# nadeemlab/DeepLIIF

Measured on AMD Instinct MI355X. Metric: 512x512 tiles/s train-step (5G+5D), higher is better.
Workload: dtype bf16; 1 GPU; DeepLIIF train step, 5x Resnet-9block G + 5x NLayerD(n=4), GAN+SmoothL1+Adam (BASELINE configs[2] per GPU); tile=512x512x3, batch_per_gpu=8, global_batch=8, norm=instance, precision_policy=bf16, parallelism=dp1, rccl_ranks=1, backend=nccl, streams=3

## Files before the change

deepliif_amd/csrc/conv_gemm.hip:

```cpp
#include "common.h"
#include <stdlib.h>

#include "conv_args.h"

bool w4_eligible(const ConvArgs &a);
int launch_conv_w4(const ConvArgs &a0, hipStream_t stream);
bool w4x3_eligible(const ConvArgs &a);
int launch_conv_w4x3(const ConvArgs &a0, hipStream_t stream);
bool s2f_eligible(const ConvArgs &a);
int s2f_stats_chunks(const ConvArgs &a);
int launch_conv_s2f(const ConvArgs &a0, hipStream_t stream);
bool d1g_eligible(const ConvArgs &a);
int launch_conv_d1g(const ConvArgs &a0, hipStream_t stream);
bool d1_eligible(const ConvArgs &a);
int launch_conv_d1(const ConvArgs &a0, hipStream_t stream);
bool dot_fwd_eligible(const ConvArgs &a);
bool dot_dgrad_eligible(const ConvArgs &a);
int launch_conv_dot(const ConvArgs &a, bool fwd, hipStream_t stream);
bool s2u_eligible(const ConvArgs &a);
int s2u_stats_chunks(const ConvArgs &a);
int launch_conv_s2u(const ConvArgs &a0, hipStream_t stream);
bool s2d_eligible(const ConvArgs &a);
int s2d_stats_chunks(const ConvArgs &a);
int launch_conv_s2d(const ConvArgs &a0, hipStream_t stream);
// ... 527 lines not shown
                    red[(wm * 2 + 0) * BN + c] = st1[i][r];
                    red[(wm * 2 + 1) * BN + c] = st2[i][r];
                }
        }
        __syncthreads();
        const int m0 = tm * BM;
        const int n = m0 / HWq;
        const int chunk = ((m0 - n * HWq) / BM) * a.n_phase + phase;
        for (int c = tid; c < BN; c += NW * 64) {
            const int co = tn * BN + c;
            if (co < a.Co) {
                float s1 = 0.f, s2 = 0.f;
#pragma unroll
                for (int w = 0; w < WM; ++w) { s1 += red[(w * 2 + 0) * BN + c]; s2 += red[(w * 2 + 1) * BN + c]; }
                float *o = a.stats_part + ((size_t)(n * a.stats_nchunks + chunk) * 2) * a.Co + co;
                o[0] = s1;
                o[a.Co] = s2;
            }
        }
    }
}


template <int BM, int BN, int BK, int WM, int WN, bool UTAP, bool STAG = false, int ABL = 0>
__global__ void __launch_bounds__(WM * WN * 64) conv_gemm_glds_kernel(const ConvArgs a) {
    constexpr int NW = WM * WN;
    constexpr int CPR = BK / 8;
    constexpr int RPI = 64 / CPR;
    constexpr int X_INS = (BM + NW * RPI - 1) / (NW * RPI);
    constexpr int W_INS = (BN + NW * RPI - 1) / (NW * RPI);
    constexpr int PM = BM / WM, PN = BN / WN, FM = PM / 16, FN = PN / 16;
    constexpr int XT = BM * BK, WT = BN * BK, BUF = XT + WT;
    static_assert(NW == 4 || NW == 8, "4 or 8 waves");

    extern __shared__ __attribute__((aligned(16))) char smem_raw[];
    bf16_t *smem = reinterpret_cast<bf16_t *>(smem_raw);
    int16_t *tap_lds = reinterpret_cast<int16_t *>(smem + 2 * BUF);
    int *tapd_lds = reinterpret_cast<int *>(tap_lds + DL_MAX_TAPS);

    const int tid = threadIdx.x;
    const int lane = tid & 63, wave = __builtin_amdgcn_readfirstlane(tid >> 6);
    const int wm = wave % WM, wn = wave / WM;

    const int bid = xcd_remap(blockIdx.x, gridDim.x);
    const int tn = bid % a.tiles_n, tm = bid / a.tiles_n;
    const int phase = blockIdx.y / a.splitk, ks = blockIdx.y % a.splitk;
    const int tap0 = a.phase_tap_begin[phase];
    const int ntaps = a.phase_tap_begin[phase + 1] - tap0;
    const int kbase = a.phase_kbase[phase];
    const int nk_total = (ntaps * a.Ci + 63) / 64 * 64 / BK;
    const int nk_per = (nk_total + a.splitk - 1) / a.splitk;
    const int kt_begin = ks * nk_per;
    const int kt_end = min(nk_total, kt_begin + nk_per);

    if (tid < DL_MAX_TAPS) {
        const int16_t tp = a.taps[tid];
        tap_lds[tid] = tp;
        tapd_lds[tid] = ((int)(int8_t)(tp & 0xff) * a.Wi + (int)(int8_t)((tp >> 8) & 0xff)) * a.in_pstride;
    }

// ... 18 lines not shown
        x_wi0[i] = wq * a.in_step;
        x_chunk[i] = swz_chunk<CPR>(row, lcp);
        x_ptr[i] = in + ((size_t)(n * a.Hi + x_hi0[i]) * a.Wi + x_wi0[i]) * (size_t)a.in_pstride + x_chunk[i] * 8;
        unsigned long long mk = 0;
        if (UTAP && x_ok[i]) {
            for (int t = 0; t < ntaps; ++t) {
                const int16_t tp = a.taps[tap0 + t];
                const int hi = x_hi0[i] + (int)(int8_t)(tp & 0xff), wi = x_wi0[i] + (int)(int8_t)((tp >> 8) & 0xff);
                if (a.pad_mode == DL_PAD_REFLECT || (((unsigned)hi < (unsigned)a.Hi) && ((unsigned)wi < (unsigned)a.Wi))) mk |= 1ull << t;
            }
        }
        x_mask[i] = mk;
    }
    const bf16_t *w_ptr[W_INS];
#pragma unroll
    for (int i = 0; i < W_INS; ++i) {
        const int row = (wave * W_INS + i) * RPI + lrow;
        const int c = swz_chunk<CPR>(row, lcp);
        w_ptr[i] = a.w_hi + (size_t)(tn * BN + (row < BN ? row : 0)) * a.w_kstride + kbase + c * 8;
    }

    int is_tl = 0, is_ch = 0;
    int tapd_next = 0;
    auto issue_tile = [&](int kt, int buf) {
        bf16_t *base = smem + buf * BUF;
        size_t wk;
        if constexpr (UTAP) {
            const int tl = is_tl;
            const ptrdiff_t delta = (ptrdiff_t)tapd_next + is_ch;
            wk = (size_t)tl * a.Ci + is_ch;
            if (a.k_order) { if (++is_tl == ntaps) { is_tl = 0; is_ch += BK; } }
            else { is_ch += BK; if (is_ch == a.Ci) { is_ch = 0; ++is_tl; } }
            tapd_next = tapd_lds[tap0 + min(is_tl, ntaps - 1)];
#pragma unroll
            for (int i = 0; i < X_INS; ++i) {
                const int row0 = (wave * X_INS + i) * RPI;
                if (row0 < BM) {
                    const bool ok = (x_mask[i] >> tl) & 1ull;
                    const bf16_t *src = ok ? x_ptr[i] + delta : zero;
                    __builtin_amdgcn_global_load_lds((const __attribute__((address_space(1))) void *)src,
                                                     (__attribute__((address_space(3))) void *)(base + row0 * BK), 16, 0, 0);
                }
            }
        } else {
            wk = (size_t)kt * BK;
#pragma unroll
            for (int i = 0; i < X_INS; ++i) {
                const int row0 = (wave * X_INS + i) * RPI;
                if (row0 < BM) {
                    const int k0 = kt * BK + x_chunk[i] * 8;
                    const int tl = k0 >> a.log2Ci;
                    const int ci = k0 & (a.Ci - 1);
                    const int tli = tl < ntaps ? tl : 0;
                    const int16_t t = tap_lds[tap0 + tli];
                    const int dh = (int)(int8_t)(t & 0xff), dw = (int)(int8_t)((t >> 8) & 0xff);
// ... 10 lines not shown
#pragma unroll
        for (int i = 0; i < W_INS; ++i) {
            const int row0 = (wave * W_INS + i) * RPI;
            if (row0 < BN) {
                __builtin_amdgcn_global_load_lds((const __attribute__((address_space(1))) void *)(w_ptr[i] + wk),
                                                 (__attribute__((address_space(3))) void *)(base + XT + row0 * BK), 16, 0, 0);
            }
        }
    };

    f32x4_t acc[FN][FM];
#pragma unroll
    for (int i = 0; i < FN; ++i)
#pragma unroll
        for (int j = 0; j < FM; ++j) acc[i][j] = f32x4_t{0.f, 0.f, 0.f, 0.f};

    __syncthreads();
    if constexpr (UTAP) {
        if (a.k_order) { is_tl = kt_begin % ntaps; is_ch = (kt_begin / ntaps) * BK; }
        else { is_tl = (kt_begin * BK) >> a.log2Ci; is_ch = (kt_begin * BK) & (a.Ci - 1); }
        tapd_next = tapd_lds[tap0 + min(is_tl, ntaps - 1)];
    }
    if (kt_begin < kt_end) issue_tile(kt_begin, 0);
    __syncthreads();

    const int fr = lane & 15, fg = lane >> 4;
    int foff[BK / 32];
#pragma unroll
    for (int kk = 0; kk < BK / 32; ++kk) foff[kk] = (fr * CPR + swz_chunk<CPR>(fr, kk * 4 + fg)) * 8;
    auto read_frags = [&](const bf16_t *Xs, const bf16_t *Ws, int kk, bf16x8_t (&wf)[FN], bf16x8_t (&xf)[FM]) {
#pragma unroll
        for (int i = 0; i < FN; ++i) wf[i] = *reinterpret_cast<const bf16x8_t *>(Ws + (wn * PN + i * 16) * BK + foff[kk]);
#pragma unroll
        for (int j = 0; j < FM; ++j) xf[j] = *reinterpret_cast<const bf16x8_t *>(Xs + (wm * PM + j * 16) * BK + foff[kk]);
    };
    auto mma = [&](const bf16x8_t (&wf)[FN], const bf16x8_t (&xf)[FM]) {
#pragma unroll
        for (int i = 0; i < FN; ++i)
#pragma unroll
            for (int j = 0; j < FM; ++j) acc[i][j] = dl_mfma16(wf[i], xf[j], acc[i][j]);
    };

    if constexpr (STAG && NW == 8 && BK == 64) {
        const bool late = wave >= 4;
        bf16x8_t wf[FN], xf[FM];
        for (int kt = kt_begin; kt < kt_end; ++kt) {
            const int cur = (kt - kt_begin) & 1;
            if (kt + 1 < kt_end) issue_tile(kt + 1, cur ^ 1);
            const bf16_t *Xs = smem + cur * BUF, *Ws = Xs + XT;
            if (late && kt > kt_begin) mma(wf, xf);
            __builtin_amdgcn_sched_barrier(0);
            read_frags(Xs, Ws, 0, wf, xf);
            __builtin_amdgcn_sched_barrier(0);
            mma(wf, xf);
            __builtin_amdgcn_sched_barrier(0);
            read_frags(Xs, Ws, 1, wf, xf);
            __builtin_amdgcn_sched_barrier(0);
            if (!late) mma(wf, xf);
            __syncthreads();
        }
        if (late && kt_begin < kt_end) mma(wf, xf);
    } else {
        for (int kt = kt_begin; kt < kt_end; ++kt) {
            const int cur = (kt - kt_begin) & 1;
            if (ABL != 1 && kt + 1 < kt_end) issue_tile(kt + 1, cur ^ 1);
            const bf16_t *Xs = smem + cur * BUF, *Ws = Xs + XT;
            if constexpr (ABL == 4) {
                asm volatile("s_waitcnt vmcnt(8)" ::: "memory");
                __builtin_amdgcn_s_barrier();
                continue;
            }
            if (ABL != 2 && ABL != 4 && ABL != 5) {
#pragma unroll
                for (int kk = 0; kk < BK / 32; ++kk) {
                    bf16x8_t wf[FN], xf[FM];
                    read_frags(Xs, Ws, kk, wf, xf);
                    mma(wf, xf);
                }
            }
            __syncthreads();
        }
    }

    glds_epilogue<BM, BN, WM, WN>(a, acc, tm, tn, phase, ks, wm, wn, lane, tid, smem_raw);
// ... 573 lines not shown
    if (a.n_phase != 1 || a.splitk != 1 || a.in_step != 1 || a.out_step != 1 || a.Wq != 128 || a.Wi != 128 || (a.Hq & 1)) return false;
    if (a.phase_tap_begin[1] - a.phase_tap_begin[0] != 9 || a.Ci < 64) return false;
    for (int kh = 0; kh < 3; ++kh) {
        const int dh0 = (int8_t)(a.taps[kh * 3] & 0xff);
        int seen = 0;
        for (int kw = 0; kw < 3; ++kw) {
            const int16_t tp = a.taps[kh * 3 + kw];
            const int dh = (int8_t)(tp & 0xff), dw = (int8_t)((tp >> 8) & 0xff);
            if (dh != dh0 || dw < -1 || dw > 1) return false;
            seen |= 1 << (dw + 1);
        }
        if (seen != 7) return false;
    }
    return true;
}

template <int ABL>
static int dispatch_p32(const ConvArgs &a, hipStream_t stream) {
    static const char *kwr_env = DL_DEV_ENV("DL_CONV_KWR");
    if (!(kwr_env && kwr_env[0] == '0') && kwr_eligible(a)) return launch_conv_p32<true, ABL>(a, stream);
    return launch_conv_p32<false, ABL>(a, stream);
}

template <int BM, int BN, int BK, int WM, int WN, bool UTAP, bool STAG = false, int ABL = 0>
static int launch_conv_glds_impl(const ConvArgs &a0, hipStream_t stream) {
    ConvArgs a = a0;
    a.tiles_m = (a.Mtot + BM - 1) / BM;
    a.tiles_n = (a.Co + BN - 1) / BN;
    constexpr size_t smem_loop = (size_t)2 * (BM + BN) * BK * sizeof(bf16_t) + DL_MAX_TAPS * (sizeof(int16_t) + sizeof(int));
    constexpr size_t smem = (BN >= 64 && epilogue_lds_bytes<BM, BN, WM>() > smem_loop) ? epilogue_lds_bytes<BM, BN, WM>() : smem_loop;
    auto kern = conv_gemm_glds_kernel<BM, BN, BK, WM, WN, UTAP, STAG, ABL>;
    static bool attr_set = false;
    if (!attr_set) {
        hipError_t e = hipFuncSetAttribute(reinterpret_cast<const void *>(kern), hipFuncAttributeMaxDynamicSharedMemorySize, (int)smem);
        if (e != hipSuccess) DL_FAIL("dl_conv_forward: hipFuncSetAttribute(%zu): %s", smem, hipGetErrorString(e));
        attr_set = true;
    }
    dim3 grid(a.tiles_m * a.tiles_n, a.n_phase * a.splitk);
    hipLaunchKernelGGL(kern, grid, dim3(WM * WN * 64), smem, stream, a);
    DL_CHECK_LAUNCH("dl_conv_forward(glds)");
    return 0;
}

template <int BM, int BN, int BK, int WM, int WN>
static int launch_conv_glds(const ConvArgs &a, hipStream_t stream) {
    if (a.Ci >= BK && a.pad_mode == DL_PAD_ZERO) return launch_conv_glds_impl<BM, BN, BK, WM, WN, true>(a, stream);
    return launch_conv_glds_impl<BM, BN, BK, WM, WN, false>(a, stream);
}

static bool big_tile_fills_gpu(int mtot, int Co, int n_phase, int splitk) {
    return Co >= 256 && (Co % 256) == 0 && (size_t)((mtot + 255) / 256) * (Co / 256) * n_phase * splitk >= 224;
}

static bool w4_enabled() {
    static const char *w4 = DL_DEV_ENV("DL_CONV_W4");
    return !(w4 && w4[0] == '0');
}

static int dispatch_tile_glds(const ConvArgs &a, hipStream_t stream) {
    if (a.Co <= 16) return launch_conv_glds<256, 16, 32, 4, 1>(a, stream);
    if (a.Co <= 64) return launch_conv_glds<128, 64, 64, 2, 2>(a, stream);
    static const bool no_big = DL_DEV_ENV("DL_NO_BIGTILE") != nullptr;
    if (!no_big && big_tile_fills_gpu(a.Mtot, a.Co, a.n_phase, a.splitk))
    {
        if (w4_enabled() && w4_eligible(a)) return launch_conv_w4(a, stream);
#ifdef DL_DEV_SWITCHES
        static const char *p32 = DL_DEV_ENV("DL_CONV_P32");
        if (p32 && p32[0] == '1' && a.Ci >= 64 && a.pad_mode == DL_PAD_ZERO && !a.k_order) {
            static const char *ablp = DL_DEV_ENV("DL_CONV_ABLATE");
            if (ablp && ablp[0] == '1') return dispatch_p32<1>(a, stream);
// ... 2 lines not shown
            return dispatch_p32<0>(a, stream);
        }
        static const char *ph8 = DL_DEV_ENV("DL_CONV_8PH");
        if (!(ph8 && ph8[0] == '0') && a.Ci >= 64 && a.pad_mode == DL_PAD_ZERO && !a.k_order) {
            static const char *abl8 = DL_DEV_ENV("DL_CONV_ABLATE");
            if (abl8 && abl8[0] == '1') return launch_conv_8ph<1>(a, stream);
            if (abl8 && abl8[0] == '2') return launch_conv_8ph<2>(a, stream);
            if (abl8 && abl8[0] == '3') return launch_conv_8ph<3>(a, stream);
            if (abl8 && abl8[0] == '4') return launch_conv_8ph<4>(a, stream);
            return launch_conv_8ph<0>(a, stream);
        }
        static const bool stag = DL_DEV_ENV("DL_CONV_STAGGER") != nullptr;
        static const char *abl = DL_DEV_ENV("DL_CONV_ABLATE");
        if (abl && abl[0] == '1' && a.Ci >= 64 && a.pad_mode == DL_PAD_ZERO) return launch_conv_glds_impl<256, 256, 64, 2, 4, true, false, 1>(a, stream);
        if (abl && abl[0] == '2' && a.Ci >= 64 && a.pad_mode == DL_PAD_ZERO) return launch_conv_glds_impl<256, 256, 64, 2, 4, true, false, 2>(a, stream);
        if (abl && abl[0] == '4' && a.Ci >= 64 && a.pad_mode == DL_PAD_ZERO) return launch_conv_glds_impl<256, 256, 64, 2, 4, true, false, 4>(a, stream);
        if (abl && abl[0] == '5' && a.Ci >= 64 && a.pad_mode == DL_PAD_ZERO) return launch_conv_glds_impl<256, 256, 64, 2, 4, true, false, 5>(a, stream);
        if (stag && a.Ci >= 64 && a.pad_mode == DL_PAD_ZERO) return launch_conv_glds_impl<256, 256, 64, 2, 4, true, true>(a, stream);
#else
        if (a.Ci >= 64 && a.pad_mode == DL_PAD_ZERO && !a.k_order) return launch_conv_8ph<0>(a, stream);
#endif
        return launch_conv_glds<256, 256, 64, 2, 4>(a, stream);
    }
    return launch_conv_glds<128, 128, 64, 2, 2>(a, stream);
}

template <typename TOut>
__global__ void __launch_bounds__(256) conv_slab_reduce_kernel(const float *slab, int splitk, size_t npix, int Co,
                                                               const float *bias, int bias_n, int act, TOut *out, int out_pstride) {
    const size_t total = npix * (size_t)(Co / 4);
    for (size_t i = blockIdx.x * (size_t)blockDim.x + threadIdx.x; i < total; i += (size_t)gridDim.x * blockDim.x) {
        const size_t p = i / (Co / 4);
        const int c = (int)(i % (Co / 4)) * 4;
        float4 s = make_float4(0, 0, 0, 0);
        for (int k = 0; k < splitk; ++k) {
            const float4 v = *reinterpret_cast<const float4 *>(slab + ((size_t)k * npix + p) * Co + c);
            s.x += v.x; s.y += v.y; s.z += v.z; s.w += v.w;
        }
        if (bias) {
            s.x += (c < bias_n) ? bias[c] : 0.f; s.y += (c + 1 < bias_n) ? bias[c + 1] : 0.f;
            s.z += (c + 2 < bias_n) ? bias[c + 2] : 0.f; s.w += (c + 3 < bias_n) ? bias[c + 3] : 0.f;
        }
        s.x = apply_act(act, s.x); s.y = apply_act(act, s.y); s.z = apply_act(act, s.z); s.w = apply_act(act, s.w);
        TOut *dst = out + p * out_pstride + c;
        store1<TOut>(dst, s.x); store1<TOut>(dst + 1, s.y); store1<TOut>(dst + 2, s.z); store1<TOut>(dst + 3, s.w);
    }
// ... 358 lines not shown
```

deepliif_amd/csrc/conv_s2f.hip:

```cpp
#include "conv_args.h"

typedef __attribute__((ext_vector_type(16))) float f32x16_t;
typedef __attribute__((address_space(3))) char lds_char_t;
typedef __attribute__((address_space(3))) const bf16x8_t lds_frag_t;

__device__ __attribute__((aligned(64))) unsigned char g_s2f_zero_page[64];

template <int V> struct S2IC { static constexpr int value = V; };

constexpr int S2F_MAX_OFF = 9;
struct S2fArgs {
    ConvArgs a;
    int n_off;
    int off_delta[S2F_MAX_OFF];
    int8_t off_dh[S2F_MAX_OFF], off_dw[S2F_MAX_OFF];
    int user_k[S2F_MAX_OFF][4];
};

__device__ __forceinline__ float s2f_row16_sum(float v) {
    v += __builtin_bit_cast(float, __builtin_amdgcn_update_dpp(0, __builtin_bit_cast(int, v), 0xB1, 0xf, 0xf, false));
    v += __builtin_bit_cast(float, __builtin_amdgcn_update_dpp(0, __builtin_bit_cast(int, v), 0x4E, 0xf, 0xf, false));
    v += __builtin_bit_cast(float, __builtin_amdgcn_update_dpp(0, __builtin_bit_cast(int, v), 0x141, 0xf, 0xf, false));
    v += __builtin_bit_cast(float, __builtin_amdgcn_update_dpp(0, __builtin_bit_cast(int, v), 0x140, 0xf, 0xf, false));
    return v;
}

constexpr int S2F_XB = 256 * 128;
constexpr int S2F_WB = 64 * 128;
constexpr int S2F_BUF = S2F_XB + 4 * S2F_WB;
constexpr size_t S2F_LOOP_LDS = (size_t)2 * S2F_BUF;
constexpr size_t S2F_EPI_LDS = (size_t)256 * 512 + 256 * sizeof(int) + (size_t)4 * 2 * 64 * sizeof(float);
constexpr size_t S2F_LDS = S2F_LOOP_LDS > S2F_EPI_LDS ? S2F_LOOP_LDS : S2F_EPI_LDS;

__global__ void __launch_bounds__(512) conv_s2f_kernel(const S2fArgs sa) {
    const ConvArgs &a = sa.a;
    extern __shared__ __attribute__((aligned(16))) char smem_raw[];
    lds_char_t *lds = (lds_char_t *)smem_raw;

    const int tid = threadIdx.x, lane = tid & 63;
    const int wave = __builtin_amdgcn_readfirstlane(tid >> 6);
    const int wm = wave & 3, wn = wave >> 2;
    const int bid = xcd_remap(blockIdx.x, gridDim.x);
    const int tn = bid % a.tiles_n, tm = bid / a.tiles_n;
    const int nch = a.Ci >> 6;
    const int NO = sa.n_off;
    const int T = nch * NO;

    const int lrow = lane >> 3, lcp = lane & 7;
    const int HWq = a.Hq * a.Wq;
    const bf16_t *in = reinterpret_cast<const bf16_t *>(a.in);
    const bf16_t *zero = reinterpret_cast<const bf16_t *>(g_s2f_zero_page);
    const bf16_t *x_ptr[4];
    unsigned x_mask[4];
#pragma unroll
    for (int i = 0; i < 4; ++i) {
        const int s = (wave * 4 + i) * 8 + lrow;
// ... 26 lines not shown
                                             (__attribute__((address_space(3))) void *)(lds + buf + (wave * 4 + i) * 1024), 16, 0, 0);
        }
#pragma unroll
        for (int p = 0; p < 4; ++p) {
            const int kb = sa.user_k[o][p];
            if (kb >= 0)
                __builtin_amdgcn_global_load_lds((const __attribute__((address_space(1))) void *)(w_ptr + kb + c * 64),
                                                 (__attribute__((address_space(3))) void *)(lds + buf + S2F_XB + p * S2F_WB + wave * 1024), 16, 0, 0);
        }
    };

    const int lr = lane & 31, lh = lane >> 5;
    const int ax = (wm * 64 + lr) * 128 + ((lh ^ ((lr >> 1) & 7)) << 4);
    const int aw = S2F_XB + (wn * 32 + lr) * 128 + ((lh ^ ((lr >> 1) & 7)) << 4);

    f32x16_t acc[4][2];
#pragma unroll
    for (int p = 0; p < 4; ++p)
#pragma unroll
        for (int j = 0; j < 2; ++j)
#pragma unroll
            for (int r = 0; r < 16; ++r) acc[p][j][r] = 0.f;

    if (T > 0) stage(0);
    for (int u = 0; u < T; ++u) {
        asm volatile("s_waitcnt vmcnt(0)\n\ts_barrier" ::: "memory");
        if (u + 1 < T) stage(u + 1);
        const int c = u / NO, o = u - c * NO;
        (void)c;
        const int buf = (u & 1) * S2F_BUF;
        bf16x8_t xf[4][2];
#pragma unroll
        for (int s = 0; s < 4; ++s)
#pragma unroll
            for (int j = 0; j < 2; ++j) xf[s][j] = *reinterpret_cast<lds_frag_t *>(lds + buf + (ax ^ (s << 5)) + j * 4096);
#pragma unroll
        for (int p = 0; p < 4; ++p) {
            if (sa.user_k[o][p] < 0) continue;
            bf16x8_t wf[4];
#pragma unroll
            for (int s = 0; s < 4; ++s) wf[s] = *reinterpret_cast<lds_frag_t *>(lds + buf + p * S2F_WB + (aw ^ (s << 5)));
#pragma unroll
            for (int s = 0; s < 4; ++s)
#pragma unroll
                for (int j = 0; j < 2; ++j) acc[p][j] = dl_mfma32(wf[s], xf[s][j], acc[p][j]);
        }
    }
    asm volatile("s_waitcnt vmcnt(0) lgkmcnt(0)" ::: "memory");
    __syncthreads();

    lds_char_t *tile = lds;
    __attribute__((address_space(3))) int *rowtab = reinterpret_cast<__attribute__((address_space(3))) int *>(lds + 256 * 512);
    __attribute__((address_space(3))) float *red = reinterpret_cast<__attribute__((address_space(3))) float *>(lds + 256 * 512 + 256 * 4);
    const bool want_stats = a.stats_part != nullptr;
    if (tid < 256) {
        const int m = tm * 256 + tid;
        int opix = -1;
        if (m < a.Mtot) {
            const int n = m / HWq, rem = m - n * HWq;
            const int hq = rem / a.Wq, wq = rem - hq * a.Wq;
            opix = (n * a.Ho + 2 * hq) * a.Wo + 2 * wq;
        }
        rowtab[tid] = opix;
    }
    bool live[2];
#pragma unroll
    for (int j = 0; j < 2; ++j) live[j] = tm * 256 + wm * 64 + j * 32 + lr < a.Mtot;
#pragma unroll
// ... 88 lines not shown
    if (a.epi_old) return false;
    const char *env = dl_switch(DL_SW_CONV_S2F);
    if (a.Mtot < 65536 && !(env && env[0] == '2')) return false;
    int ndist = 0;
    int16_t seen[S2F_MAX_OFF + 1];
    for (int t = 0; t < a.phase_tap_begin[4]; ++t) {
        bool dup = false;
        for (int i = 0; i < ndist; ++i) dup |= seen[i] == a.taps[t];
        if (!dup) {
            if (ndist == S2F_MAX_OFF) return false;
            seen[ndist++] = a.taps[t];
        }
    }
    for (int p = 0; p < 4; ++p)
        for (int t = a.phase_tap_begin[p]; t < a.phase_tap_begin[p + 1]; ++t)
            for (int t2 = t + 1; t2 < a.phase_tap_begin[p + 1]; ++t2)
                if (a.taps[t] == a.taps[t2]) return false;
    return ndist > 0;
}

int s2f_stats_chunks(const ConvArgs &a) {
    const int hw = a.Hq * a.Wq;
    return (hw % 256) ? 0 : hw / 256;
}

int launch_conv_s2f(const ConvArgs &a0, hipStream_t stream) {
    S2fArgs sa;
    memset(&sa, 0, sizeof(sa));
    sa.a = a0;
    ConvArgs &a = sa.a;
    a.tiles_m = (a.Mtot + 255) / 256;
    a.tiles_n = a.Co / 64;
    int no = 0;
    int16_t key[S2F_MAX_OFF];
    for (int p = 0; p < 4; ++p)
        for (int t = a.phase_tap_begin[p]; t < a.phase_tap_begin[p + 1]; ++t) {
            int o = -1;
            for (int i = 0; i < no; ++i)
                if (key[i] == a.taps[t]) o = i;
            if (o < 0) {
                o = no++;
                key[o] = a.taps[t];
                sa.off_dh[o] = (int8_t)(a.taps[t] & 0xff);
                sa.off_dw[o] = (int8_t)((a.taps[t] >> 8) & 0xff);
                sa.off_delta[o] = ((int)sa.off_dh[o] * a.Wi + (int)sa.off_dw[o]) * a.in_pstride;
                for (int q = 0; q < 4; ++q) sa.user_k[o][q] = -1;
            }
            sa.user_k[o][p] = a.phase_kbase[p] + (t - a.phase_tap_begin[p]) * a.Ci;
        }
    sa.n_off = no;
    static bool attr_set = false;
    if (!attr_set) {
        hipError_t e = hipFuncSetAttribute(reinterpret_cast<const void *>(conv_s2f_kernel), hipFuncAttributeMaxDynamicSharedMemorySize, (int)S2F_LDS);
        if (e != hipSuccess) DL_FAIL("dl_conv_forward(s2f): hipFuncSetAttribute(%zu): %s", S2F_LDS, hipGetErrorString(e));
        attr_set = true;
    }
    dim3 grid(a.tiles_m * a.tiles_n, 1);
    hipLaunchKernelGGL(conv_s2f_kernel, grid, dim3(512), S2F_LDS, stream, sa);
    DL_CHECK_LAUNCH("dl_conv_forward(s2f)");
    return 0;
}
```

deepliif_amd/csrc/wgrad.hip:

```cpp
#include "common.h"
#include <stdlib.h>

typedef __attribute__((ext_vector_type(4))) short s16x4_t;

struct WgradArgs {
    const void *P;
    const void *Q;
    float *slab;
    int kstride;
    int N, Hp, Wp, CAp, p_pstride;
    int Hq, Wq, CBp, log2CB, q_pstride;
    int KH, KW, step, pad, pad_w, pad_mode;
    int J;
    int Ptot;
    int splitk, pchunk;
    int tiles_a, tiles_j;
    int dn, dh, dw;
    int p_act, q_act;
    int xcd_group;
    int p_split, q_split;
    int tr_asm;
};

constexpr int WGRAD_MULTI_MAX = DL_WGRAD_MULTI_MAX;
// ... 238 lines not shown
}

template <int ROWB>
__device__ __forceinline__ bf16x8_t tr_fragment_swz_asm(const bf16_t *tile, int prow0, int slot, int lane) {
    const int m = lane & 15, g = lane >> 4;
    const int x = (m >> 2) | ((g & 1) << 2);
    const char *base = reinterpret_cast<const char *>(tile) + (prow0 + 8 * g + (m >> 2)) * ROWB + ((slot ^ x) << 5) + (m & 3) * 8;
    const uint32_t addr = (uint32_t)(uintptr_t)(__attribute__((address_space(3))) const char *)base;
    s16x4_t lo, hi;
    asm volatile("ds_read_b64_tr_b16 %0, %1" : "=v"(lo) : "v"(addr) : "memory");
    asm volatile("ds_read_b64_tr_b16 %0, %1 offset:%2" : "=v"(hi) : "v"(addr), "n"(4 * ROWB) : "memory");
    bf16x8_t r;
    r[0] = lo[0]; r[1] = lo[1]; r[2] = lo[2]; r[3] = lo[3];
    r[4] = hi[0]; r[5] = hi[1]; r[6] = hi[2]; r[7] = hi[3];
    return r;
}
__device__ __forceinline__ void tr_wait4(bf16x8_t (&f)[4]) {
    asm volatile("s_waitcnt lgkmcnt(0)" : "+v"(f[0]), "+v"(f[1]), "+v"(f[2]), "+v"(f[3]) : : "memory");
}
__device__ __forceinline__ void tr_wait8(bf16x8_t (&f)[8]) {
    asm volatile("s_waitcnt lgkmcnt(0)" : "+v"(f[0]), "+v"(f[1]), "+v"(f[2]), "+v"(f[3]), "+v"(f[4]), "+v"(f[5]), "+v"(f[6]), "+v"(f[7]) : : "memory");
}

template <int BA, int WA, int WJ, bool TRASM>
__global__ void __launch_bounds__(512) wgrad_glds_kernel(const WgradArgs a, const WgradLayers lay) {
    constexpr int BJ = 256, BP = 64, NW = 8;
    constexpr int PA = BA / WA, PJ = BJ / WJ, FA = PA / 16, FJ = PJ / 16;
    constexpr int ROWA = BA * 2, ROWJ = BJ * 2;
    constexpr int TA = BP * BA, TJ = BP * BJ, BUF = TA + TJ;
    constexpr int A_RPI = 1024 / ROWA, J_RPI = 1024 / ROWJ;
    constexpr int A_INS = BP / (NW * A_RPI), J_INS = BP / (NW * J_RPI);
    static_assert(WA * WJ == NW, "8 waves");
    static_assert(A_INS >= 1 && J_INS >= 1, "tile too small for 8 waves");

    extern __shared__ __attribute__((aligned(16))) char smem_raw[];
    bf16_t *smem = reinterpret_cast<bf16_t *>(smem_raw);

    const int tid = threadIdx.x, lane = tid & 63, wave = __builtin_amdgcn_readfirstlane(tid >> 6);
    const int wa = wave % WA, wj = wave / WA;
    int bid, ks, layer;
    if (a.xcd_group) {
        const int ntile = gridDim.x;
        const int logical = xcd_remap((blockIdx.z * gridDim.y + blockIdx.y) * ntile + blockIdx.x, ntile * gridDim.y * gridDim.z);
        const int grp = logical / ntile;
        bid = logical - grp * ntile;
        layer = grp / gridDim.y;
        ks = grp - layer * gridDim.y;
    } else {
        bid = xcd_remap(blockIdx.x, gridDim.x);
// ... 54 lines not shown
#pragma unroll
        for (int i = 0; i < J_INS; ++i) {
            const int h = q_h[i] * a.step - a.pad + q_kh[i], w = q_w[i] * a.step - a.pad_w + q_kw[i];
            const bool ok = q_tap_ok[i] && (pbase + q_row[i] < p_end) && ((unsigned)h < (unsigned)a.Hq) && ((unsigned)w < (unsigned)a.Wq);
            const bf16_t *src = ok ? Q + ((size_t)(q_n[i] * a.Hq + h) * a.Wq + w) * a.q_pstride + q_cb[i] : zero;
            __builtin_amdgcn_global_load_lds((const __attribute__((address_space(1))) void *)src,
                                             (__attribute__((address_space(3))) void *)(base + TA + (wave * J_INS + i) * J_RPI * BJ), 16, 0, 0);
            q_w[i] += a.dw;
            const int cw = q_w[i] >= a.Wp;
            q_w[i] -= cw ? a.Wp : 0;
            q_h[i] += a.dh + cw;
            const int chh = q_h[i] >= a.Hp;
            q_h[i] -= chh ? a.Hp : 0;
            q_n[i] += a.dn + chh;
        }
    };

    f32x4_t acc[FA][FJ];
#pragma unroll
    for (int i = 0; i < FA; ++i)
#pragma unroll
        for (int j = 0; j < FJ; ++j) acc[i][j] = f32x4_t{0.f, 0.f, 0.f, 0.f};

    if (nk > 0) issue_tile(0, 0);
    __syncthreads();

    for (int kt = 0; kt < nk; ++kt) {
        const int cur = kt & 1;
        if (kt + 1 < nk) issue_tile(kt + 1, cur ^ 1);
        const bf16_t *Ps = smem + cur * BUF, *Qs = Ps + TA;
#pragma unroll
        for (int ss = 0; ss < BP / 32; ++ss) {
            bf16x8_t af[FA], bf[FJ];
            static_assert(FJ == 4 && (FA == 8 || FA == 4), "fragment counts of the explicit waits");
            if constexpr (TRASM) {
#pragma unroll
                for (int i = 0; i < FA; ++i) af[i] = tr_fragment_swz_asm<ROWA>(Ps, ss * 32, (wa * PA) / 16 + i, lane);
#pragma unroll
                for (int j = 0; j < FJ; ++j) bf[j] = tr_fragment_swz_asm<ROWJ>(Qs, ss * 32, (wj * PJ) / 16 + j, lane);
                if constexpr (FA == 8) tr_wait8(af); else tr_wait4(*reinterpret_cast<bf16x8_t (*)[4]>(&af[0]));
                tr_wait4(bf);
            } else {
#pragma unroll
                for (int i = 0; i < FA; ++i) af[i] = tr_fragment_swz<ROWA>(Ps, ss * 32, (wa * PA) / 16 + i, lane);
#pragma unroll
                for (int j = 0; j < FJ; ++j) bf[j] = tr_fragment_swz<ROWJ>(Qs, ss * 32, (wj * PJ) / 16 + j, lane);
            }
#pragma unroll
            for (int i = 0; i < FA; ++i)
#pragma unroll
                for (int j = 0; j < FJ; ++j) acc[i][j] = dl_mfma16(af[i], bf[j], acc[i][j]);
        }
        __syncthreads();
    }

    const int fr = lane & 15, fg = lane >> 4;
#pragma unroll
    for (int i = 0; i < FA; ++i)
#pragma unroll
        for (int j = 0; j < FJ; ++j) {
            const int jj = tj * BJ + wj * PJ + j * 16 + fr;
            if (jj >= a.J) continue;
#pragma unroll
            for (int r = 0; r < 4; ++r) {
                const int ca = ta * BA + wa * PA + i * 16 + fg * 4 + r;
                if (ca < a.CAp) slab[(size_t)ks * a.kstride + (size_t)ca * a.J + jj] = acc[i][j][r];
            }
        }
}

#define DL_WBAR() asm volatile("s_barrier" ::: "memory")
template <int V> struct IC { static constexpr int value = V; };
__global__ void __launch_bounds__(512) wgrad_8ph_kernel(const WgradArgs a) {
    constexpr int BA = 256, BJ = 256, BP = 64, HP = 32;
    constexpr int ROWA = BA * 2, ROWJ = BJ * 2;
    constexpr int TA = BP * BA, TJ = BP * BJ, BUF = TA + TJ;

// ... 169 lines not shown
                if (ca < a.CAp) a.slab[(size_t)ks * a.kstride + (size_t)ca * a.J + jj] = acc[i][j][r];
            }
        }
}

static int launch_wgrad_8ph(WgradArgs a, hipStream_t stream) {
    constexpr size_t smem = (size_t)2 * 64 * (256 + 256) * sizeof(bf16_t);
    a.tiles_a = a.CAp / 256;
    a.tiles_j = (a.J + 255) / 256;
    a.pchunk = ((a.Ptot + a.splitk - 1) / a.splitk + 63) / 64 * 64;
    const int hw = a.Hp * a.Wp;
    a.dn = 64 / hw; a.dh = (64 % hw) / a.Wp; a.dw = (64 % hw) % a.Wp;
    static bool attr_set = false;
    if (!attr_set) {
        hipError_t e = hipFuncSetAttribute(reinterpret_cast<const void *>(wgrad_8ph_kernel), hipFuncAttributeMaxDynamicSharedMemorySize, (int)smem);
        if (e != hipSuccess) DL_FAIL("dl_conv_wgrad: hipFuncSetAttribute: %s", hipGetErrorString(e));
        attr_set = true;
    }
    hipLaunchKernelGGL(wgrad_8ph_kernel, dim3(a.tiles_a * a.tiles_j, a.splitk), dim3(512), smem, stream, a);
    DL_CHECK_LAUNCH("dl_conv_wgrad(8-phase)");
    return 0;
}

template <int BA, int WA, int WJ, bool TRASM>
static int launch_wgrad_glds_v(WgradArgs a, const WgradLayers &lay, int n, hipStream_t stream) {
    constexpr size_t smem = (size_t)2 * 64 * (BA + 256) * sizeof(bf16_t);
    a.tiles_a = a.CAp / BA;
    a.tiles_j = (a.J + 255) / 256;
    a.pchunk = ((a.Ptot + a.splitk - 1) / a.splitk + 63) / 64 * 64;
    const int hw = a.Hp * a.Wp;
    a.dn = 64 / hw; a.dh = (64 % hw) / a.Wp; a.dw = (64 % hw) % a.Wp;
    auto kern = wgrad_glds_kernel<BA, WA, WJ, TRASM>;
    static bool attr_set = false;
    if (!attr_set) {
        hipError_t e = hipFuncSetAttribute(reinterpret_cast<const void *>(kern), hipFuncAttributeMaxDynamicSharedMemorySize, (int)smem);
        if (e != hipSuccess) DL_FAIL("dl_conv_wgrad: hipFuncSetAttribute: %s", hipGetErrorString(e));
        attr_set = true;
    }
    hipLaunchKernelGGL(kern, dim3(a.tiles_a * a.tiles_j, a.splitk, n), dim3(512), smem, stream, a, lay);
    DL_CHECK_LAUNCH("dl_conv_wgrad(glds)");
    return 0;
}

template <int BA, int WA, int WJ>
static int launch_wgrad_glds(const WgradArgs &a, const WgradLayers &lay, int n, hipStream_t stream) {
    return a.tr_asm ? launch_wgrad_glds_v<BA, WA, WJ, true>(a, lay, n, stream) : launch_wgrad_glds_v<BA, WA, WJ, false>(a, lay, n, stream);
}

__device__ __forceinline__ void wgrad_reduce_body(const float *slab, int splitk, int kstride_, int CBp, int J, int CA, int CB, int KK, float *grad,
                                                  int accumulate, int stack_kw, int bid, int nb) {
    const int J4 = J / 4;
    const size_t total = (size_t)CA * J4;
    const size_t kstride = (size_t)kstride_;
    for (size_t i = bid * (size_t)blockDim.x + threadIdx.x; i < total; i += (size_t)nb * blockDim.x) {
        const int ca = (int)(i / J4), j = (int)(i % J4) * 4;
        const float *src = slab + (size_t)ca * J + j;
        f32x4_t s = {0.f, 0.f, 0.f, 0.f};
        int k = 0;
        for (; k + 8 <= splitk; k += 8) {
            f32x4_t v[8];
#pragma unroll
            for (int u = 0; u < 8; ++u) v[u] = __builtin_nontemporal_load(reinterpret_cast<const f32x4_t *>(src + (size_t)(k + u) * kstride));
#pragma unroll
            for (int u = 0; u < 8; ++u) s += v[u];
        }
        for (; k < splitk; ++k) s += __builtin_nontemporal_load(reinterpret_cast<const f32x4_t *>(src + (size_t)k * kstride));
        const int t = j / CBp, b0 = j % CBp;
        if (t >= KK) continue;
#pragma unroll
// ... 324 lines not shown
```

Measured before the change: 118.9 tiles/s.

## Add multi-stage LDS ring pipelines to conv, s2f and wgrad GEMM kernels

Adds 3- and 4-stage LDS ring buffers with explicit vmcnt-based waits to the conv glds kernel, the s2f kernel and the wgrad glds kernel. The goal is to keep more global-to-LDS loads in flight so memory latency overlaps with MFMA work. The rings are gated behind dev environment switches. The default wgrad path is also restructured into one waitcnt+barrier per k-step instead of two barriers, and the tap/channel advance in conv issue_tile becomes branchless. The extra stages use more LDS, which can lower occupancy, and the hand-written waitcnt counts must match the number of issued loads exactly.

```diff
diff --git a/deepliif_amd/csrc/conv_gemm.hip b/deepliif_amd/csrc/conv_gemm.hip
--- a/deepliif_amd/csrc/conv_gemm.hip
+++ b/deepliif_amd/csrc/conv_gemm.hip
@@ -573,7 +573,7 @@
 }
 
 
-template <int BM, int BN, int BK, int WM, int WN, bool UTAP, bool STAG = false, int ABL = 0>
+template <int BM, int BN, int BK, int WM, int WN, bool UTAP, bool STAG = false, int ABL = 0, int NS = 2>
 __global__ void __launch_bounds__(WM * WN * 64) conv_gemm_glds_kernel(const ConvArgs a) {
     constexpr int NW = WM * WN;
     constexpr int CPR = BK / 8;
@@ -586,7 +586,7 @@
 
     extern __shared__ __attribute__((aligned(16))) char smem_raw[];
     bf16_t *smem = reinterpret_cast<bf16_t *>(smem_raw);
-    int16_t *tap_lds = reinterpret_cast<int16_t *>(smem + 2 * BUF);
+    int16_t *tap_lds = reinterpret_cast<int16_t *>(smem + NS * BUF);
     int *tapd_lds = reinterpret_cast<int *>(tap_lds + DL_MAX_TAPS);
 
     const int tid = threadIdx.x;
@@ -651,15 +651,20 @@
 
     int is_tl = 0, is_ch = 0;
     int tapd_next = 0;
-    auto issue_tile = [&](int kt, int buf) {
+    auto issue_tile = [&](int kt, int buf) __attribute__((always_inline)) {
         bf16_t *base = smem + buf * BUF;
         size_t wk;
         if constexpr (UTAP) {
             const int tl = is_tl;
             const ptrdiff_t delta = (ptrdiff_t)tapd_next + is_ch;
             wk = (size_t)tl * a.Ci + is_ch;
-            if (a.k_order) { if (++is_tl == ntaps) { is_tl = 0; is_ch += BK; } }
-            else { is_ch += BK; if (is_ch == a.Ci) { is_ch = 0; ++is_tl; } }
+            {
+                const bool ko = a.k_order != 0;
+                const int tl1 = is_tl + 1, ch1 = is_ch + BK;
+                const bool wrap = ko ? (tl1 == ntaps) : (ch1 == a.Ci);
+                is_tl = ko ? (wrap ? 0 : tl1) : (wrap ? tl1 : is_tl);
+                is_ch = ko ? (wrap ? ch1 : is_ch) : (wrap ? 0 : ch1);
+            }
             tapd_next = tapd_lds[tap0 + min(is_tl, ntaps - 1)];
 #pragma unroll
             for (int i = 0; i < X_INS; ++i) {
@@ -716,7 +721,7 @@
         tapd_next = tapd_lds[tap0 + min(is_tl, ntaps - 1)];
     }
     if (kt_begin < kt_end) issue_tile(kt_begin, 0);
-    __syncthreads();
+    if constexpr (NS == 2) __syncthreads();
 
     const int fr = lane & 15, fg = lane >> 4;
     int foff[BK / 32];
@@ -754,6 +759,30 @@
             __syncthreads();
         }
         if (late && kt_begin < kt_end) mma(wf, xf);
+    } else if constexpr (NS > 2) {
+        static_assert(NS <= 4 && ABL == 0 && BM % (NW * RPI) == 0 && BN % (NW * RPI) == 0, "ring: every wave issues X_INS + W_INS instructions per stage");
+        constexpr int INS = X_INS + W_INS;
+#pragma unroll
+        for (int s = 1; s < NS - 1; ++s)
+            if (kt_begin + s < kt_end) issue_tile(kt_begin + s, s);
+        int cur = 0, nxt = NS - 1;
+        for (int kt = kt_begin; kt < kt_end; ++kt) {
+            const int younger = kt_end - 1 - kt;
+            if (younger >= NS - 2) asm volatile("s_waitcnt vmcnt(%0) lgkmcnt(0)\n\ts_barrier" : : "n"((NS - 2) * INS) : "memory");
+            else if (NS == 4 && younger == 1) asm volatile("s_waitcnt vmcnt(%0) lgkmcnt(0)\n\ts_barrier" : : "n"(INS) : "memory");
+            else asm volatile("s_waitcnt vmcnt(0) lgkmcnt(0)\n\ts_barrier" ::: "memory");
+            if (kt + NS - 1 < kt_end) issue_tile(kt + NS - 1, nxt);
+            const bf16_t *Xs = smem + cur * BUF, *Ws = Xs + XT;
+#pragma unroll
+            for (int kk = 0; kk < BK / 32; ++kk) {
+                bf16x8_t wf[FN], xf[FM];
+                read_frags(Xs, Ws, kk, wf, xf);
+                mma(wf, xf);
+            }
+            cur = (cur + 1 == NS) ? 0 : cur + 1;
+            nxt = (nxt + 1 == NS) ? 0 : nxt + 1;
+        }
+        __syncthreads();
     } else {
         for (int kt = kt_begin; kt < kt_end; ++kt) {
             const int cur = (kt - kt_begin) & 1;
@@ -1373,14 +1402,15 @@
     return launch_conv_p32<false, ABL>(a, stream);
 }
 
-template <int BM, int BN, int BK, int WM, int WN, bool UTAP, bool STAG = false, int ABL = 0>
+template <int BM, int BN, int BK, int WM, int WN, bool UTAP, bool STAG = false, int ABL = 0, int NS = 2>
 static int launch_conv_glds_impl(const ConvArgs &a0, hipStream_t stream) {
     ConvArgs a = a0;
     a.tiles_m = (a.Mtot + BM - 1) / BM;
     a.tiles_n = (a.Co + BN - 1) / BN;
-    constexpr size_t smem_loop = (size_t)2 * (BM + BN) * BK * sizeof(bf16_t) + DL_MAX_TAPS * (sizeof(int16_t) + sizeof(int));
+    constexpr size_t smem_loop = (size_t)NS * (BM + BN) * BK * sizeof(bf16_t) + DL_MAX_TAPS * (sizeof(int16_t) + sizeof(int));
     constexpr size_t smem = (BN >= 64 && epilogue_lds_bytes<BM, BN, WM>() > smem_loop) ? epilogue_lds_bytes<BM, BN, WM>() : smem_loop;
-    auto kern = conv_gemm_glds_kernel<BM, BN, BK, WM, WN, UTAP, STAG, ABL>;
+    static_assert(smem <= 160 * 1024, "LDS budget");
+    auto kern = conv_gemm_glds_kernel<BM, BN, BK, WM, WN, UTAP, STAG, ABL, NS>;
     static bool attr_set = false;
     if (!attr_set) {
         hipError_t e = hipFuncSetAttribute(reinterpret_cast<const void *>(kern), hipFuncAttributeMaxDynamicSharedMemorySize, (int)smem);
@@ -1393,10 +1423,10 @@
     return 0;
 }
 
-template <int BM, int BN, int BK, int WM, int WN>
+template <int BM, int BN, int BK, int WM, int WN, int NS = 2>
 static int launch_conv_glds(const ConvArgs &a, hipStream_t stream) {
-    if (a.Ci >= BK && a.pad_mode == DL_PAD_ZERO) return launch_conv_glds_impl<BM, BN, BK, WM, WN, true>(a, stream);
-    return launch_conv_glds_impl<BM, BN, BK, WM, WN, false>(a, stream);
+    if (a.Ci >= BK && a.pad_mode == DL_PAD_ZERO) return launch_conv_glds_impl<BM, BN, BK, WM, WN, true, false, 0, NS>(a, stream);
+    return launch_conv_glds_impl<BM, BN, BK, WM, WN, false, false, 0, NS>(a, stream);
 }
 
 static bool big_tile_fills_gpu(int mtot, int Co, int n_phase, int splitk) {
@@ -1445,6 +1475,10 @@
 #endif
         return launch_conv_glds<256, 256, 64, 2, 4>(a, stream);
     }
+#ifdef DL_DEV_SWITCHES
+    static const char *ring = DL_DEV_ENV("DL_CONV_RING");
+    if (ring && ring[0] == '1') return launch_conv_glds<128, 128, 64, 2, 2, 3>(a, stream);
+#endif
     return launch_conv_glds<128, 128, 64, 2, 2>(a, stream);
 }
 
diff --git a/deepliif_amd/csrc/conv_s2f.hip b/deepliif_amd/csrc/conv_s2f.hip
--- a/deepliif_amd/csrc/conv_s2f.hip
+++ b/deepliif_amd/csrc/conv_s2f.hip
@@ -15,6 +15,7 @@
     int off_delta[S2F_MAX_OFF];
     int8_t off_dh[S2F_MAX_OFF], off_dw[S2F_MAX_OFF];
     int user_k[S2F_MAX_OFF][4];
+    unsigned nw_packed;
 };
 
 __device__ __forceinline__ float s2f_row16_sum(float v) {
@@ -28,10 +29,16 @@
 constexpr int S2F_XB = 256 * 128;
 constexpr int S2F_WB = 64 * 128;
 constexpr int S2F_BUF = S2F_XB + 4 * S2F_WB;
-constexpr size_t S2F_LOOP_LDS = (size_t)2 * S2F_BUF;
+constexpr int S2F_NX = 3, S2F_NW = 8;
+constexpr int S2F_WOFF = S2F_NX * S2F_XB;
 constexpr size_t S2F_EPI_LDS = (size_t)256 * 512 + 256 * sizeof(int) + (size_t)4 * 2 * 64 * sizeof(float);
-constexpr size_t S2F_LDS = S2F_LOOP_LDS > S2F_EPI_LDS ? S2F_LOOP_LDS : S2F_EPI_LDS;
-
+template <bool RING> constexpr size_t s2f_lds_bytes() {
+    constexpr size_t loop = RING ? (size_t)S2F_NX * S2F_XB + (size_t)S2F_NW * S2F_WB : (size_t)2 * S2F_BUF;
+    return loop > S2F_EPI_LDS ? loop : S2F_EPI_LDS;
+}
+static_assert(s2f_lds_bytes<true>() <= 160 * 1024, "LDS budget");
+
+template <bool RING>
 __global__ void __launch_bounds__(512) conv_s2f_kernel(const S2fArgs sa) {
     const ConvArgs &a = sa.a;
     extern __shared__ __attribute__((aligned(16))) char smem_raw[];
@@ -104,28 +111,88 @@
 #pragma unroll
             for (int r = 0; r < 16; ++r) acc[p][j][r] = 0.f;
 
-    if (T > 0) stage(0);
-    for (int u = 0; u < T; ++u) {
-        asm volatile("s_waitcnt vmcnt(0)\n\ts_barrier" ::: "memory");
-        if (u + 1 < T) stage(u + 1);
-        const int c = u / NO, o = u - c * NO;
-        (void)c;
-        const int buf = (u & 1) * S2F_BUF;
-        bf16x8_t xf[4][2];
-#pragma unroll
-        for (int s = 0; s < 4; ++s)
-#pragma unroll
-            for (int j = 0; j < 2; ++j) xf[s][j] = *reinterpret_cast<lds_frag_t *>(lds + buf + (ax ^ (s << 5)) + j * 4096);
-#pragma unroll
-        for (int p = 0; p < 4; ++p) {
-            if (sa.user_k[o][p] < 0) continue;
-            bf16x8_t wf[4];
-#pragma unroll
-            for (int s = 0; s < 4; ++s) wf[s] = *reinterpret_cast<lds_frag_t *>(lds + buf + p * S2F_WB + (aw ^ (s << 5)));
+    if constexpr (RING) {
+        int so = 0, sc = 0, sx = 0, sw = 0;
+        auto stage_ring = [&]() __attribute__((always_inline)) {
+            const ptrdiff_t xd = (ptrdiff_t)sa.off_delta[so] + sc * 64;
+#pragma unroll
+            for (int i = 0; i < 4; ++i) {
+                const bool ok = (x_mask[i] >> so) & 1u;
+                const bf16_t *src = ok ? x_ptr[i] + xd : zero;
+                __builtin_amdgcn_global_load_lds((const __attribute__((address_space(1))) void *)src,
+                                                 (__attribute__((address_space(3))) void *)(lds + sx * S2F_XB + (wave * 4 + i) * 1024), 16, 0, 0);
+            }
+#pragma unroll
+            for (int p = 0; p < 4; ++p) {
+                const int kb = sa.user_k[so][p];
+                if (kb >= 0) {
+                    __builtin_amdgcn_global_load_lds((const __attribute__((address_space(1))) void *)(w_ptr + kb + sc * 64),
+                                                     (__attribute__((address_space(3))) void *)(lds + S2F_WOFF + sw * S2F_WB + wave * 1024), 16, 0, 0);
+                    sw = (sw + 1) & (S2F_NW - 1);
+                }
+            }
+            sx = (sx + 1 == S2F_NX) ? 0 : sx + 1;
+            if (++so == NO) { so = 0; ++sc; }
+        };
+        if (T > 0) stage_ring();
+        if (T > 1) stage_ring();
+        int ro = 0, rx = 0, rw = 0;
+        for (int u = 0; u < T; ++u) {
+            const int on = (ro + 1 == NO) ? 0 : ro + 1;
+            const int keep = (u + 1 < T) ? 4 + (int)((sa.nw_packed >> (3 * on)) & 7u) : 0;
+            switch (keep) {
+                case 5: asm volatile("s_waitcnt vmcnt(5) lgkmcnt(0)\n\ts_barrier" ::: "memory"); break;
+                case 6: asm volatile("s_waitcnt vmcnt(6) lgkmcnt(0)\n\ts_barrier" ::: "memory"); break;
+                case 7: asm volatile("s_waitcnt vmcnt(7) lgkmcnt(0)\n\ts_barrier" ::: "memory"); break;
+                case 8: asm volatile("s_waitcnt vmcnt(8) lgkmcnt(0)\n\ts_barrier" ::: "memory"); break;
+                default: asm volatile("s_waitcnt vmcnt(0) lgkmcnt(0)\n\ts_barrier" ::: "memory"); break;
+            }
+            if (u + 2 < T) stage_ring();
+            const int bufx = rx * S2F_XB;
+            bf16x8_t xf[4][2];
 #pragma unroll
             for (int s = 0; s < 4; ++s)
 #pragma unroll
-                for (int j = 0; j < 2; ++j) acc[p][j] = dl_mfma32(wf[s], xf[s][j], acc[p][j]);
+                for (int j = 0; j < 2; ++j) xf[s][j] = *reinterpret_cast<lds_frag_t *>(lds + bufx + (ax ^ (s << 5)) + j * 4096);
+#pragma unroll
+            for (int p = 0; p < 4; ++p) {
+                if (sa.user_k[ro][p] < 0) continue;
+                bf16x8_t wf[4];
+#pragma unroll
+                for (int s = 0; s < 4; ++s) wf[s] = *reinterpret_cast<lds_frag_t *>(lds + S2F_WOFF + rw * S2F_WB + ((aw - S2F_XB) ^ (s << 5)));
+                rw = (rw + 1) & (S2F_NW - 1);
+#pragma unroll
+                for (int s = 0; s < 4; ++s)
+#pragma unroll
+                    for (int j = 0; j < 2; ++j) acc[p][j] = dl_mfma32(wf[s], xf[s][j], acc[p][j]);
+            }
+            rx = (rx + 1 == S2F_NX) ? 0 : rx + 1;
+            ro = on;
+        }
+    } else {
+        if (T > 0) stage(0);
+        for (int u = 0; u < T; ++u) {
+            asm volatile("s_waitcnt vmcnt(0)\n\ts_barrier" ::: "memory");
+            if (u + 1 < T) stage(u + 1);
+            const int c = u / NO, o = u - c * NO;
+            (void)c;
+            const int buf = (u & 1) * S2F_BUF;
+            bf16x8_t xf[4][2];
+    #pragma unroll
+            for (int s = 0; s < 4; ++s)
+    #pragma unroll
+                for (int j = 0; j < 2; ++j) xf[s][j] = *reinterpret_cast<lds_frag_t *>(lds + buf + (ax ^ (s << 5)) + j * 4096);
+    #pragma unroll
+            for (int p = 0; p < 4; ++p) {
+                if (sa.user_k[o][p] < 0) continue;
+                bf16x8_t wf[4];
+    #pragma unroll
+                for (int s = 0; s < 4; ++s) wf[s] = *reinterpret_cast<lds_frag_t *>(lds + buf + p * S2F_WB + (aw ^ (s << 5)));
+    #pragma unroll
+                for (int s = 0; s < 4; ++s)
+    #pragma unroll
+                    for (int j = 0; j < 2; ++j) acc[p][j] = dl_mfma32(wf[s], xf[s][j], acc[p][j]);
+            }
         }
     }
     asm volatile("s_waitcnt vmcnt(0) lgkmcnt(0)" ::: "memory");
@@ -260,6 +327,21 @@
 int s2f_stats_chunks(const ConvArgs &a) {
     const int hw = a.Hq * a.Wq;
     return (hw % 256) ? 0 : hw / 256;
+}
+
+template <bool RING>
+static int launch_conv_s2f_v(const S2fArgs &sa, hipStream_t stream) {
+    constexpr size_t lds_bytes = s2f_lds_bytes<RING>();
+    static bool attr_set = false;
+    if (!attr_set) {
+        hipError_t e = hipFuncSetAttribute(reinterpret_cast<const void *>(conv_s2f_kernel<RING>), hipFuncAttributeMaxDynamicSharedMemorySize, (int)lds_bytes);
+        if (e != hipSuccess) DL_FAIL("dl_conv_forward(s2f): hipFuncSetAttribute(%zu): %s", lds_bytes, hipGetErrorString(e));
+        attr_set = true;
+    }
+    dim3 grid(sa.a.tiles_m * sa.a.tiles_n, 1);
+    hipLaunchKernelGGL(conv_s2f_kernel<RING>, grid, dim3(512), lds_bytes, stream, sa);
+    DL_CHECK_LAUNCH("dl_conv_forward(s2f)");
+    return 0;
 }
 
 int launch_conv_s2f(const ConvArgs &a0, hipStream_t stream) {
@@ -287,14 +369,19 @@
             sa.user_k[o][p] = a.phase_kbase[p] + (t - a.phase_tap_begin[p]) * a.Ci;
         }
     sa.n_off = no;
-    static bool attr_set = false;
-    if (!attr_set) {
-        hipError_t e = hipFuncSetAttribute(reinterpret_cast<const void *>(conv_s2f_kernel), hipFuncAttributeMaxDynamicSharedMemorySize, (int)S2F_LDS);
-        if (e != hipSuccess) DL_FAIL("dl_conv_forward(s2f): hipFuncSetAttribute(%zu): %s", S2F_LDS, hipGetErrorString(e));
-        attr_set = true;
-    }
-    dim3 grid(a.tiles_m * a.tiles_n, 1);
-    hipLaunchKernelGGL(conv_s2f_kernel, grid, dim3(512), S2F_LDS, stream, sa);
-    DL_CHECK_LAUNCH("dl_conv_forward(s2f)");
-    return 0;
-}
+#ifdef DL_DEV_SWITCHES
+    static const char *ring = DL_DEV_ENV("DL_S2F_RING");
+    if (ring && ring[0] == '1') {
+        int nw[S2F_MAX_OFF];
+        bool fits = true;
+        for (int o = 0; o < no; ++o) {
+            nw[o] = 0;
+            for (int q = 0; q < 4; ++q) nw[o] += sa.user_k[o][q] >= 0;
+            sa.nw_packed |= (unsigned)nw[o] << (3 * o);
+        }
+        for (int o = 0; o < no; ++o) fits &= nw[o] + nw[(o + 1) % no] + nw[(o + 2) % no] <= S2F_NW;
+        if (fits) return launch_conv_s2f_v<true>(sa, stream);
+    }
+#endif
+    return launch_conv_s2f_v<false>(sa, stream);
+}
diff --git a/deepliif_amd/csrc/wgrad.hip b/deepliif_amd/csrc/wgrad.hip
--- a/deepliif_amd/csrc/wgrad.hip
+++ b/deepliif_amd/csrc/wgrad.hip
@@ -284,9 +284,9 @@
     asm volatile("s_waitcnt lgkmcnt(0)" : "+v"(f[0]), "+v"(f[1]), "+v"(f[2]), "+v"(f[3]), "+v"(f[4]), "+v"(f[5]), "+v"(f[6]), "+v"(f[7]) : : "memory");
 }
 
-template <int BA, int WA, int WJ, bool TRASM>
+template <int BA, int WA, int WJ, bool TRASM, int BP = 64, int NS = 2>
 __global__ void __launch_bounds__(512) wgrad_glds_kernel(const WgradArgs a, const WgradLayers lay) {
-    constexpr int BJ = 256, BP = 64, NW = 8;
+    constexpr int BJ = 256, NW = 8;
     constexpr int PA = BA / WA, PJ = BJ / WJ, FA = PA / 16, FJ = PJ / 16;
     constexpr int ROWA = BA * 2, ROWJ = BJ * 2;
     constexpr int TA = BP * BA, TJ = BP * BJ, BUF = TA + TJ;
@@ -387,12 +387,16 @@
 #pragma unroll
         for (int j = 0; j < FJ; ++j) acc[i][j] = f32x4_t{0.f, 0.f, 0.f, 0.f};
 
-    if (nk > 0) issue_tile(0, 0);
-    __syncthreads();
-
+    static_assert(NS >= 2 && NS <= 4 && (BP == 32 || BP == 64), "ring geometry");
+    constexpr int KEEP = (NS - 2) * (A_INS + J_INS);
+    if (nk > 0) {
+#pragma unroll
+        for (int s = 0; s < NS - 1; ++s) issue_tile(s, s);
+    }
+    int cur = 0, nxt = NS - 1;
     for (int kt = 0; kt < nk; ++kt) {
-        const int cur = kt & 1;
-        if (kt + 1 < nk) issue_tile(kt + 1, cur ^ 1);
+        asm volatile("s_waitcnt vmcnt(%0) lgkmcnt(0)\n\ts_barrier" : : "n"(KEEP) : "memory");
+        issue_tile(kt + NS - 1, nxt);
         const bf16_t *Ps = smem + cur * BUF, *Qs = Ps + TA;
 #pragma unroll
         for (int ss = 0; ss < BP / 32; ++ss) {
@@ -416,8 +420,10 @@
 #pragma unroll
                 for (int j = 0; j < FJ; ++j) acc[i][j] = dl_mfma16(af[i], bf[j], acc[i][j]);
         }
-        __syncthreads();
-    }
+        cur = (cur + 1 == NS) ? 0 : cur + 1;
+        nxt = (nxt + 1 == NS) ? 0 : nxt + 1;
+    }
+    asm volatile("s_waitcnt vmcnt(0)" ::: "memory");
 
     const int fr = lane & 15, fg = lane >> 4;
 #pragma unroll
@@ -633,15 +639,16 @@
     return 0;
 }
 
-template <int BA, int WA, int WJ, bool TRASM>
+template <int BA, int WA, int WJ, bool TRASM, int BP, int NS>
 static int launch_wgrad_glds_v(WgradArgs a, const WgradLayers &lay, int n, hipStream_t stream) {
-    constexpr size_t smem = (size_t)2 * 64 * (BA + 256) * sizeof(bf16_t);
+    constexpr size_t smem = (size_t)NS * BP * (BA + 256) * sizeof(bf16_t);
+    static_assert(smem <= 160 * 1024, "LDS budget");
     a.tiles_a = a.CAp / BA;
     a.tiles_j = (a.J + 255) / 256;
     a.pchunk = ((a.Ptot + a.splitk - 1) / a.splitk + 63) / 64 * 64;
     const int hw = a.Hp * a.Wp;
-    a.dn = 64 / hw; a.dh = (64 % hw) / a.Wp; a.dw = (64 % hw) % a.Wp;
-    auto kern = wgrad_glds_kernel<BA, WA, WJ, TRASM>;
+    a.dn = BP / hw; a.dh = (BP % hw) / a.Wp; a.dw = (BP % hw) % a.Wp;
+    auto kern = wgrad_glds_kernel<BA, WA, WJ, TRASM, BP, NS>;
     static bool attr_set = false;
     if (!attr_set) {
         hipError_t e = hipFuncSetAttribute(reinterpret_cast<const void *>(kern), hipFuncAttributeMaxDynamicSharedMemorySize, (int)smem);
@@ -655,7 +662,14 @@
 
 template <int BA, int WA, int WJ>
 static int launch_wgrad_glds(const WgradArgs &a, const WgradLayers &lay, int n, hipStream_t stream) {
-    return a.tr_asm ? launch_wgrad_glds_v<BA, WA, WJ, true>(a, lay, n, stream) : launch_wgrad_glds_v<BA, WA, WJ, false>(a, lay, n, stream);
+#ifdef DL_DEV_SWITCHES
+    static const char *ring_env = DL_DEV_ENV("DL_WGRAD_RING");
+    if (ring_env && ring_env[0] == '1') {
+        constexpr int BP = BA == 256 ? 32 : 64, NS = BA == 256 ? 4 : 3;
+        return a.tr_asm ? launch_wgrad_glds_v<BA, WA, WJ, true, BP, NS>(a, lay, n, stream) : launch_wgrad_glds_v<BA, WA, WJ, false, BP, NS>(a, lay, n, stream);
+    }
+#endif
+    return a.tr_asm ? launch_wgrad_glds_v<BA, WA, WJ, true, 64, 2>(a, lay, n, stream) : launch_wgrad_glds_v<BA, WA, WJ, false, 64, 2>(a, lay, n, stream);
 }
 
 __device__ __forceinline__ void wgrad_reduce_body(const float *slab, int splitk, int kstride_, int CBp, int J, int CA, int CB, int KK, float *grad,
```

Result: no change. 119.2 tiles/s (median of 6 runs) (+0.2%).
